# ai-forever/Kandinsky-2

Measured on NVIDIA H100. Metric: unet_denoising_steps_per_sec, higher is better.
Workload: dtype f16

## Files before the change

### kandinsky-2_b200/csrc/k2_api.cu

```cuda
#include <stdio.h>
#include <stdlib.h>
#include <string.h>

#include <algorithm>
#include <atomic>
#include <mutex>

#include "../../include/k2b200.h"
#include "k2_internal.h"

namespace k2 {

static thread_local std::string g_err;
static std::atomic<long long> g_launches{0};
static int g_force_bn = 0;
static int g_force_split = 0;
static int g_pdl = 0;


void set_error(const std::string& msg) { g_err = msg; }
int fail(const std::string& msg) {
  g_err = msg;
  return -1;
}
// ... 74 lines not shown
      const int th = static_cast<int>((H + tiles_h - 1) / tiles_h);
      const long long tiles = tiles_h * tiles_w * ((NB + tn - 1) / tn);
      for (int k = (tn == 1 ? 0 : 1); k < 2; ++k) {
        bool better = best_tiles[k] < 0 || tiles < best_tiles[k];
        if (!better && tiles == best_tiles[k]) {
          if (tn != bn[k]) {
            better = tn < bn[k];
          } else {
            const int d_new = tw > th ? tw - th : th - tw;
            const int d_old = bw[k] > bh[k] ? bw[k] - bh[k] : bh[k] - bw[k];
            better = (d_new < d_old) || (d_new == d_old && tw > bw[k]);
          }
        }
        if (better) {
          best_tiles[k] = tiles;
          bn[k] = tn;
          bw[k] = tw;
          bh[k] = th;
        }
      }
    }
  }
  const int k = (!single_image_only && best_tiles[1] * 100 <= best_tiles[0] * 85) ? 1 : 0;
  TN = bn[k];
  TW = bw[k];
  TH = bh[k];
}


struct ConvPlan {
  int TN, TH, TW, tiles_w, tiles_h, tiles_n, m_tiles;
  int m_tiles_phase;
  int BN, splits;
  int fuse_stats, row_groups;
};

static void plan_conv(int NB, int H, int W, bool any9, int kchunks, int Cout, int out_mode, bool has_workspace,
                      long long workspace_bytes, bool want_gn, ConvPlan& pl, const int* cfg = nullptr, bool up2 = false,
                      bool w_batched = false) {
  const int g_force_bn = (cfg && cfg[0]) ? cfg[0] : k2::g_force_bn;
  const int g_force_split = (cfg && cfg[2]) ? cfg[2] : k2::g_force_split;
  choose_tile(NB, H, W, pl.TN, pl.TH, pl.TW, w_batched);
  pl.tiles_w = (W + pl.TW - 1) / pl.TW;
  pl.tiles_h = (H + pl.TH - 1) / pl.TH;
  pl.tiles_n = (NB + pl.TN - 1) / pl.TN;
  pl.m_tiles = pl.tiles_w * pl.tiles_h * pl.tiles_n;
  pl.m_tiles_phase = pl.m_tiles;

  int BN = g_force_bn;
  int splits = 1;
  const long long M_total = static_cast<long long>(NB) * H * W;
  const bool can_split = !up2 && !w_batched && has_workspace && out_mode == 0 && Cout % 8 == 0;
  auto split_ok = [&](int sp) {
    if (sp == 1) return true;
    const int kps = (kchunks + sp - 1) / sp;
    return can_split && kps >= 8 && (sp - 1) * kps < kchunks &&
           static_cast<long long>(sp) * M_total * Cout * 4 <= workspace_bytes;
  };
  auto model = [&](int bn, int sp) {
    const long long nt = (Cout + bn - 1) / bn;
    const long long units = static_cast<long long>(pl.m_tiles) * nt * sp * (up2 ? 4 : 1);
    const long long slots = num_sms();
    const long long waves = (units + slots - 1) / slots;
    const long long kps = (kchunks + sp - 1) / sp;
    long long cost = waves * (kps * (4LL * bn + 60) + 2000);
    if (sp > 1) cost += 4000 + (static_cast<long long>(sp) + 1) * M_total * Cout * 4 / 1800;
    return cost;
  };
  if (BN == 0) {
    if (Cout <= 16) BN = 16;
    else if (Cout <= 64) BN = 64;
    else if (Cout <= 128) BN = 128;
    else BN = 0;
  }
  {
    const int cand[3] = {256, 192, 128};
    long long best = -1;
    int best_bn = BN ? BN : 256, best_sp = 1;
    for (int ci = 0; ci < 3; ++ci) {
      const int bn = BN ? BN : cand[ci];
      if (BN && ci > 0) break;
      for (int sp = 1; sp <= 8; ++sp) {
        if (g_force_split > 0 && sp != g_force_split) continue;
        if (!split_ok(sp)) continue;
        const long long c = model(bn, sp);
        if (best < 0 || c < best) {
          best = c;
          best_bn = bn;
          best_sp = sp;
        }
      }
    }
    BN = best_bn;
    splits = best_sp;
  }
  pl.BN = BN;
  pl.splits = splits;

  pl.fuse_stats = 0;
  pl.row_groups = 0;
  if (want_gn && out_mode == 0 && Cout % 8 == 0) {
    if (splits == 1 && BN >= 64 && Cout % 64 == 0 && (pl.TN == 1 || pl.TH * pl.TW == 16)) {
      pl.fuse_stats = 1;
      pl.row_groups = ((pl.TN == 1) ? pl.m_tiles : NB * pl.tiles_h * pl.tiles_w) * (up2 ? 4 : 1);
    } else if (splits > 1 && (static_cast<long long>(H) * W) % 16 == 0) {
      pl.fuse_stats = 2;
      pl.row_groups = static_cast<int>(M_total / 16);
    }
  }
}

static void plan_to_info(const ConvPlan& pl, int* info) {
  if (!info) return;
  info[0] = pl.BN; info[1] = 0;
  info[2] = pl.splits; info[3] = pl.m_tiles; info[4] = pl.TN;
  info[5] = pl.fuse_stats; info[6] = pl.row_groups;
}

}

using namespace k2;

extern "C" {

const char* k2_last_error(void) { return g_err.c_str(); }
int k2_version(void) { return 100; }
long long k2_launch_count(void) { return g_launches.load(); }
void k2_reset_launch_count(void) { g_launches.store(0); }
int k2_set_tuning(int key, int value) {
  if (key == 0) {
// ... 16 lines not shown
    return 0;
  }
  if (key == 11) {
    g_gn_bps = value;
    return 0;
  }
  if (key == 9) {
    return 0;
  }

  return fail("k2_set_tuning: unknown key");
}

int k2_conv_gemm(const K2ConvSrc* srcs, int nsrc, int NB, int H, int W, const void* w_packed, int w_rows,
                 int Ktot, int ldw, int Cout, const float* bias, const void* residual, int ldr, void* out, int ldo,
                 int out_mode, void* workspace, long long workspace_bytes, float* gn_partial, int* info,
                 k2_stream_t stream) {
  return k2_conv_gemm_cfg(srcs, nsrc, NB, H, W, w_packed, w_rows, Ktot, ldw, Cout, bias, residual, ldr, out, ldo, out_mode,
                          workspace, workspace_bytes, gn_partial, info, nullptr, 0, stream);
}

int k2_conv_gemm_cfg(const K2ConvSrc* srcs, int nsrc, int NB, int H, int W, const void* w_packed, int w_rows,
                     int Ktot, int ldw, int Cout, const float* bias, const void* residual, int ldr, void* out, int ldo,
                     int out_mode, void* workspace, long long workspace_bytes, float* gn_partial, int* info,
                     const int* cfg, long long w_batch_stride, k2_stream_t stream) {
  K2_REQUIRE(w_batch_stride >= 0 && w_batch_stride % 8 == 0, "conv_gemm_cfg: w_batch_stride must be a multiple of 8 elements");
  K2_REQUIRE(out_mode == 0 || out_mode == 1, "conv_gemm: out_mode must be 0 (fp16 rows) or 1 (fp32 NCHW)");
  K2_REQUIRE(out_mode == 0 || residual == nullptr, "conv_gemm: out_mode 1 (fp32 NCHW) takes no residual");
  const bool w_batched = w_batch_stride > 0;
  if (cfg) {
    K2_REQUIRE(cfg[0] == 0 || cfg[0] == 16 || cfg[0] == 64 || cfg[0] == 128 || cfg[0] == 192 || cfg[0] == 256,
               "conv_gemm_cfg: N tile must be 0, 16, 64, 128, 192 or 256");
    K2_REQUIRE(cfg[1] >= 0 && cfg[1] <= 2 && cfg[2] >= 0 && cfg[2] <= 8 && cfg[3] >= 0 && cfg[3] <= 2,
               "conv_gemm_cfg: pair mode in 0..2, splits in 0..8, epilogue sets in 0..2");
    K2_REQUIRE(cfg[1] != 2, "conv_gemm_cfg: no CTA-pair conv kernel on sm_90");
  }
  K2_REQUIRE(nsrc >= 1 && nsrc <= 3, "conv_gemm: 1..3 sources");
  K2_REQUIRE((reinterpret_cast<uintptr_t>(gn_partial) & 7) == 0, "conv_gemm: gn_partial must be 8-byte aligned");
  K2_REQUIRE(NB > 0 && H > 0 && W > 0 && Cout > 0, "conv_gemm: bad geometry");
  K2_REQUIRE(w_rows >= Cout, "conv_gemm: w_rows < Cout");
  K2_REQUIRE(Ktot % 64 == 0, "conv_gemm: Ktot must be a multiple of 64");
  if (ldw == 0) ldw = Ktot;
  K2_REQUIRE(ldw >= Ktot && ldw % 8 == 0 && (reinterpret_cast<uintptr_t>(w_packed) & 15) == 0,
             "conv_gemm: weight row stride / alignment");
  ConvGemmParams p;
  memset(&p, 0, sizeof p);
  p.NB = NB;
  p.H = H;
  p.W = W;
  bool any9 = false;
  int kchunks = 0;
  const bool up2 = srcs[0].taps == 4;
  if (up2) {
    K2_REQUIRE(nsrc == 1 && out_mode == 0 && residual == nullptr && H % 2 == 0 && W % 2 == 0,
               "conv_gemm: a taps == 4 source (3x3 conv over its nearest-2x upsampling) must be the only source, with fp16 "
               "output, no residual and even output H, W");
    H /= 2;
    W /= 2;
    p.H = H;
    p.W = W;
  }
  for (int s = 0; s < nsrc; ++s) {
    const K2ConvSrc& src = srcs[s];
    K2_REQUIRE(src.taps == 9 || src.taps == 1 || (s == 0 && src.taps == 4), "conv_gemm: taps must be 9 or 1 (or 4: up2)");
    K2_REQUIRE(src.C > 0 && src.C % 8 == 0 && src.ld % 8 == 0 && src.ld >= src.C, "conv_gemm: bad source C/ld");
    K2_REQUIRE((reinterpret_cast<uintptr_t>(src.ptr) & 15) == 0, "conv_gemm: source not 16B aligned");
    any9 = any9 || src.taps == 9;
// ... 27 lines not shown
                        static_cast<uint64_t>(NB)};
    uint64_t str[3] = {static_cast<uint64_t>(src.ld) * 2, static_cast<uint64_t>(src.ld) * 2 * W,
                       static_cast<uint64_t>(src.ld) * 2 * W * H};
    uint32_t box[4] = {64, static_cast<uint32_t>(p.TW), static_cast<uint32_t>(p.TH), static_cast<uint32_t>(p.TN)};
    if (encode_tmap_f16(&p.tmA[s], src.ptr, 4, dims, str, box)) return -1;
  }
  const int BN = pl.BN, splits = pl.splits, fuse_stats = pl.fuse_stats;
  p.splits = splits;
  p.k_per_split = (kchunks + splits - 1) / splits;
  p.M_total = static_cast<long long>(NB) * H * W * (up2 ? 4 : 1);
  p.ws = reinterpret_cast<float*>(workspace);
  p.n_tiles = (Cout + BN - 1) / BN;
  p.Cout = Cout;
  {
    uint64_t dims[3] = {static_cast<uint64_t>(Ktot), static_cast<uint64_t>(w_rows), static_cast<uint64_t>(w_batched ? NB : 1)};
    uint64_t str[2] = {static_cast<uint64_t>(ldw) * 2,
                       (w_batched ? static_cast<uint64_t>(w_batch_stride) : static_cast<uint64_t>(ldw) * w_rows) * 2};
    uint32_t box[3] = {64, static_cast<uint32_t>(BN), 1};
    if (encode_tmap_f16(&p.tmB, w_packed, 3, dims, str, box)) return -1;
  }
  p.bias = bias;
  p.residual = reinterpret_cast<const __half*>(residual);
  p.ldr = ldr;
  p.out = out;
  p.ldo = ldo;
  p.out_mode = (splits > 1) ? 2 : out_mode;
  p.gn_part = (fuse_stats == 1) ? reinterpret_cast<float2*>(gn_partial) : nullptr;
  p.gn_mode = (fuse_stats == 1) ? (p.TN == 1 ? 1 : 2) : 0;
  if (out_mode == 0) {
    K2_REQUIRE(ldo % 8 == 0 && (reinterpret_cast<uintptr_t>(out) & 15) == 0, "conv_gemm: out alignment");
    if (residual)
      K2_REQUIRE(ldr % 8 == 0 && (reinterpret_cast<uintptr_t>(residual) & 15) == 0, "conv_gemm: residual alignment");
  }
  int rc = launch_conv_gemm(p, BN, static_cast<cudaStream_t>(stream));
  if (rc == 0) g_launches.fetch_add(1, std::memory_order_relaxed);
  if (rc == 0 && splits > 1) {
    rc = launch_splitk_finalize(p.ws, splits, p.M_total, Cout, bias, p.residual, ldr, reinterpret_cast<__half*>(out), ldo,
                                fuse_stats == 2 ? reinterpret_cast<float2*>(gn_partial) : nullptr,
                                static_cast<cudaStream_t>(stream));
    if (rc == 0) g_launches.fetch_add(1, std::memory_order_relaxed);
  }
  return rc;
}

int k2_conv_plan(int NB, int H, int W, int taps, int Ktot, int Cout, int out_mode, long long workspace_bytes,
                 int want_gn_partial, int* info) {
  K2_REQUIRE(NB > 0 && H > 0 && W > 0 && Cout > 0 && info, "conv_plan: bad arguments");
  K2_REQUIRE(Ktot > 0 && Ktot % 64 == 0, "conv_plan: Ktot must be a positive multiple of 64");
  ConvPlan pl;
  plan_conv(NB, H, W, taps == 9, Ktot / 64, Cout, out_mode, workspace_bytes > 0, workspace_bytes, want_gn_partial != 0, pl);
  plan_to_info(pl, info);
  return 0;
}

}
```

### kandinsky-2_b200/csrc/k2_conv_gemm.cu

```cuda
#include <stdio.h>

#include "k2_common.cuh"
#include "k2_internal.h"

namespace k2 {

namespace {

constexpr int BM = 128;
constexpr int BK = 64;
constexpr int A_STAGE_BYTES = BM * BK * 2;
constexpr int EPI_WARP_BYTES = 16 * 128;
constexpr int SMEM_LIMIT = 227 * 1024;

template <int BN>
struct Cfg {
  static constexpr int B_STAGE_BYTES = BN * BK * 2;
  static constexpr int STAGE_BYTES = A_STAGE_BYTES + B_STAGE_BYTES;
  static constexpr int EPI_BYTES = 8 * (EPI_WARP_BYTES + BN * 4);
  static constexpr int BAR_BYTES = 256;
  static constexpr int FIXED = EPI_BYTES + BAR_BYTES + 1024;
  static constexpr int STAGES = (SMEM_LIMIT - FIXED) / STAGE_BYTES > 6 ? 6 : (SMEM_LIMIT - FIXED) / STAGE_BYTES;
  static constexpr int SMEM_BYTES = STAGES * STAGE_BYTES + FIXED;
  static_assert(STAGES >= 2, "conv_gemm: shared memory does not hold two pipeline stages");
};

__device__ __forceinline__ void decode_m_tile(const ConvGemmParams& p, int m_idx, int& n0, int& y0,
                                              int& x0, int& phase) {
  phase = 0;
  if (p.up2) {
    phase = m_idx / p.m_tiles_phase;
    m_idx -= phase * p.m_tiles_phase;
  }
  int tw_i = m_idx % p.tiles_w;
  int t = m_idx / p.tiles_w;
  int th_i = t % p.tiles_h;
  int tn_i = t / p.tiles_h;
  x0 = tw_i * p.TW;
  y0 = th_i * p.TH;
  n0 = tn_i * p.TN;
}

__device__ __forceinline__ void ldsm_x4(uint32_t (&r)[4], uint32_t saddr) {
  asm volatile("ldmatrix.sync.aligned.m8n8.x4.shared.b16 {%0, %1, %2, %3}, [%4];"
               : "=r"(r[0]), "=r"(r[1]), "=r"(r[2]), "=r"(r[3])
               : "r"(saddr)
               : "memory");
}

template <int BN>
__device__ __forceinline__ void epilogue_warp(const ConvGemmParams& p, const float (&acc)[BN / 2], float* epi, uint32_t stg,
                                              const float* bsm, int k, int lane, int n0, int y0, int x0, int cbase, int split,
                                              int m_idx, int phase) {
  const int thw = p.TH * p.TW;
  auto out_row_of = [&](int row, int& n, int& y, int& x) -> long long {
    const int tn = row / thw;
    const int rem = row - tn * thw;
    const int th = rem / p.TW;
    const int tw = rem - th * p.TW;
    n = n0 + tn;
    y = y0 + th;
    x = x0 + tw;
    if (tn >= p.TN || n >= p.NB || y >= p.H || x >= p.W) return -1;
    return p.up2 ? (static_cast<long long>(n) * (2 * p.H) + (2 * y + (phase >> 1))) * (2 * p.W) + (2 * x + (phase & 1))
                 : (static_cast<long long>(n) * p.H + y) * p.W + x;
  };
  const int t4 = lane & 3, ra = lane >> 2;
  if constexpr (BN % 64 == 0) {
    if ((p.out_mode == 0 && p.Cout % 64 == 0) || (p.out_mode == 2 && p.Cout % 32 == 0)) {
      int n_, y_, x_;
      const int my_pix = static_cast<int>(out_row_of(16 * k + (lane & 15), n_, y_, x_));
      const int sub = lane >> 3, piece = lane & 7;
      int pix[4];
#pragma unroll
      for (int i = 0; i < 4; ++i) pix[i] = __shfl_sync(0xffffffffu, my_pix, 4 * i + sub);
      const bool va = __shfl_sync(0xffffffffu, my_pix, ra) >= 0, vb = __shfl_sync(0xffffffffu, my_pix, ra + 8) >= 0;
      auto row_addr = [&](int i) {
        const int rr = 4 * i + sub;
        return stg + rr * 128 + ((piece ^ (rr & 7)) << 4);
      };
      const int lrow = (lane & 7) + 8 * ((lane >> 3) & 1);
      auto frag_addr = [&](int q) { return stg + lrow * 128 + (((q + (lane >> 4)) ^ (lane & 7)) << 4); };
      if (p.out_mode == 2) {
        float* wsb = p.ws + static_cast<long long>(split) * p.M_total * p.Cout;
#pragma unroll
        for (int j = 0; j < BN / 32; ++j) {
          const int col0 = cbase + j * 32;
          if (col0 >= p.Cout) break;
#pragma unroll
          for (int q = 0; q < 4; ++q) {
#pragma unroll
            for (int h = 0; h < 2; ++h) {
              const int rr = ra + 8 * h;
              const int i = 16 * j + 4 * q + 2 * h;
              sts_v2(stg + rr * 128 + (((2 * q + (t4 >> 1)) ^ (rr & 7)) << 4) + ((t4 & 1) << 3), __float_as_uint(acc[i]),
                     __float_as_uint(acc[i + 1]));
            }
          }
          __syncwarp();
#pragma unroll
          for (int i = 0; i < 4; ++i) {
            const uint4 v4 = lds_v4(row_addr(i));
            if (pix[i] >= 0)
              *reinterpret_cast<uint4*>(wsb + static_cast<long long>(pix[i]) * p.Cout + col0 + piece * 4) = v4;
          }
          __syncwarp();
        }
        return;
      }
      constexpr int NP = BN / 64;
      const int m_in = p.up2 ? m_idx - phase * p.m_tiles_phase : m_idx;
      auto part_index = [&](long long base) { return p.up2 ? base * 4 + phase : base; };
      __half* outb = reinterpret_cast<__half*>(p.out);
      float4 st[NP];
      uint4 rpre[4];
      auto load_res = [&](int j) {
        const int c0 = cbase + j * 64;
#pragma unroll
        for (int i = 0; i < 4; ++i) {
          rpre[i] = make_uint4(0u, 0u, 0u, 0u);
          if (pix[i] >= 0 && c0 < p.Cout)
            rpre[i] = *reinterpret_cast<const uint4*>(p.residual + static_cast<long long>(pix[i]) * p.ldr + c0 + piece * 8);
        }
      };
      if (p.residual) load_res(0);
#pragma unroll
      for (int j = 0; j < NP; ++j) {
        const int col0 = cbase + j * 64;
        st[j] = make_float4(0.f, 0.f, 0.f, 0.f);
        if (col0 >= p.Cout) continue;
        uint32_t res[16];
        if (p.residual) {
#pragma unroll
          for (int i = 0; i < 4; ++i) sts_v4(row_addr(i), rpre[i].x, rpre[i].y, rpre[i].z, rpre[i].w);
          __syncwarp();
#pragma unroll
          for (int qq = 0; qq < 4; ++qq) {
            uint32_t r4[4];
            ldsm_x4(r4, frag_addr(2 * qq));
#pragma unroll
            for (int m = 0; m < 4; ++m) res[4 * qq + m] = r4[m];
          }
          if (j + 1 < NP) load_res(j + 1);
          __syncwarp();
        }
        uint32_t o[16];
#pragma unroll
// ... 16 lines not shown
          }
        }
#pragma unroll
        for (int qq = 0; qq < 4; ++qq) stmatrix_x4(frag_addr(2 * qq), o[4 * qq], o[4 * qq + 1], o[4 * qq + 2], o[4 * qq + 3]);
        __syncwarp();
#pragma unroll
        for (int i = 0; i < 4; ++i) {
          const uint4 v4 = lds_v4(row_addr(i));
          if (pix[i] >= 0) *reinterpret_cast<uint4*>(outb + static_cast<long long>(pix[i]) * p.ldo + col0 + piece * 8) = v4;
        }
        if (p.gn_part) {
          float4 hs = make_float4(0.f, 0.f, 0.f, 0.f);
#pragma unroll
          for (int rr = 0; rr < 16; ++rr) {
            const uint32_t v = lds_u32(stg + rr * 128 + (((lane >> 2) ^ (rr & 7)) << 4) + ((lane & 3) << 2));
            const float2 t = __half22float2(*reinterpret_cast<const __half2*>(&v));
            hs.x += t.x;
            hs.y = fmaf(t.x, t.x, hs.y);
            hs.z += t.y;
            hs.w = fmaf(t.y, t.y, hs.w);
          }
          if (p.gn_mode == 2) {
            const int per = p.tiles_h * p.tiles_w;
            const int sp = m_in % per;
            const int img = n0 + k;
            if (k < p.TN && img < p.NB)
              *reinterpret_cast<float4*>(p.gn_part + part_index(static_cast<long long>(img) * per + sp) * p.Cout + col0 + 2 * lane) = hs;
          } else {
            st[j] = hs;
          }
        }
        __syncwarp();
      }
      if (p.gn_part && p.gn_mode == 1) {
        float4* sums = reinterpret_cast<float4*>(epi);
#pragma unroll
        for (int j = 0; j < NP; ++j) sums[k * 128 + j * 32 + lane] = st[j];
        named_bar_sync(1, 256);
        if (k < NP && cbase + k * 64 < p.Cout) {
          float4 tot = make_float4(0.f, 0.f, 0.f, 0.f);
#pragma unroll
          for (int e = 0; e < 4; ++e) {
            const float4 a = sums[(2 * e) * 128 + k * 32 + lane], b = sums[(2 * e + 1) * 128 + k * 32 + lane];
            tot.x += a.x + b.x;
            tot.y += a.y + b.y;
            tot.z += a.z + b.z;
            tot.w += a.w + b.w;
          }
          *reinterpret_cast<float4*>(p.gn_part + part_index(m_in) * p.Cout + cbase + k * 64 + 2 * lane) = tot;
        }
        named_bar_sync(1, 256);
      }
      return;
    }
  }
  int n[2], y[2], x[2];
  long long orow[2];
#pragma unroll
  for (int h = 0; h < 2; ++h) orow[h] = out_row_of(16 * k + ra + 8 * h, n[h], y[h], x[h]);
#pragma unroll
  for (int q = 0; q < BN / 8; ++q) {
#pragma unroll
    for (int h = 0; h < 2; ++h) {
#pragma unroll
      for (int e = 0; e < 2; ++e) {
        const int col = cbase + 8 * q + 2 * t4 + e;
        if (orow[h] < 0 || col >= p.Cout) continue;
        float f = acc[4 * q + 2 * h + e];
        if (p.out_mode == 2) {
          p.ws[(static_cast<long long>(split) * p.M_total + orow[h]) * p.Cout + col] = f;
          continue;
        }
        if (p.bias) f += __ldg(p.bias + col);
        if (p.out_mode == 0) {
          if (p.residual) f += __half2float(p.residual[orow[h] * p.ldr + col]);
          reinterpret_cast<__half*>(p.out)[orow[h] * p.ldo + col] = __float2half_rn(f);
        } else {
          reinterpret_cast<float*>(p.out)[((static_cast<long long>(n[h]) * p.Cout + col) * p.H + y[h]) * p.W + x[h]] = f;
        }
      }
    }
  }
}


template <int BN>
__global__ void __launch_bounds__(384, 1) conv_gemm_kernel(const __grid_constant__ ConvGemmParams p) {
  using C = Cfg<BN>;
  constexpr int NA = BN / 2;
  extern __shared__ uint8_t smem_raw[];
  uint8_t* smem = reinterpret_cast<uint8_t*>((reinterpret_cast<uintptr_t>(smem_raw) + 1023) &
                                             ~static_cast<uintptr_t>(1023));
  float* epi = reinterpret_cast<float*>(smem + C::STAGES * C::STAGE_BYTES);
  uint64_t* full_bar = reinterpret_cast<uint64_t*>(smem + C::STAGES * C::STAGE_BYTES + C::EPI_BYTES);
  uint64_t* empty_bar = full_bar + C::STAGES;

  const int warp_idx = threadIdx.x >> 5;
  const int lane = threadIdx.x & 31;
  const int wg = warp_idx >> 2;

  if (threadIdx.x == 0) {
    tma_prefetch_desc(&p.tmB);
    for (int s = 0; s < 3; ++s)
      if (p.seg_taps[s]) tma_prefetch_desc(&p.tmA[s]);
    for (int i = 0; i < C::STAGES; ++i) {
      mbar_init(&full_bar[i], 1);
      mbar_init(&empty_bar[i], 8);
    }
    fence_barrier_init();
  }
  __syncthreads();
  pdl_wait();
  pdl_launch();

  const int total_tiles = p.m_tiles * p.n_tiles * p.splits;

  if (wg == 0) {
    setmaxnreg_dec<40>();
    if (warp_idx == 0 && elect_one()) {
      int stage = 0;
      uint32_t ring_phase = 0;
      const uint32_t tx_bytes = p.a_box_bytes + C::B_STAGE_BYTES;
      for (int tile = blockIdx.x; tile < total_tiles; tile += gridDim.x) {
        const int n_idx = tile % p.n_tiles;
        const int m_idx = (tile / p.n_tiles) % p.m_tiles;
        const int split = tile / (p.m_tiles * p.n_tiles);
        int n0, y0, x0, phase;
        decode_m_tile(p, m_idx, n0, y0, x0, phase);
        const int kb = phase * p.num_k_chunks;
        const int k0 = split * p.k_per_split;
        const int k1 = min(p.num_k_chunks, k0 + p.k_per_split);
        int s = 0, rem = k0;
        while (rem >= p.seg_taps[s] * p.seg_kchunks[s]) {
          rem -= p.seg_taps[s] * p.seg_kchunks[s];
          ++s;
        }
        int tap = rem / p.seg_kchunks[s];
        int c = rem - tap * p.seg_kchunks[s];
        for (int kc = k0; kc < k1; ++kc) {
          const int taps = p.seg_taps[s];
          const int dy = (taps == 9) ? (tap / 3 - 1) : (taps == 4 ? (tap >> 1) + (phase >> 1) - 1 : 0);
          const int dx = (taps == 9) ? (tap % 3 - 1) : (taps == 4 ? (tap & 1) + (phase & 1) - 1 : 0);
          mbar_wait_lean(&empty_bar[stage], ring_phase ^ 1);
          uint8_t* sA = smem + stage * C::STAGE_BYTES;
          uint8_t* sB = sA + A_STAGE_BYTES;
          mbar_arrive_expect_tx(&full_bar[stage], tx_bytes);
          tma_load_4d(sA, &p.tmA[s], &full_bar[stage], c * BK, x0 + dx, y0 + dy, n0);
          tma_load_3d(sB, &p.tmB, &full_bar[stage], (kb + kc) * BK, n_idx * BN, p.w_batched ? n0 : 0);
          if (++stage == C::STAGES) {
            stage = 0;
            ring_phase ^= 1;
          }
          if (++c == p.seg_kchunks[s]) {
            c = 0;
            if (++tap == taps) {
              tap = 0;
              ++s;
            }
          }
        }
      }
    }
  } else {
    setmaxnreg_inc<232>();
    const int g = wg - 1;
    const int k = warp_idx - 4;
    const uint32_t stg = smem_u32(epi) + k * EPI_WARP_BYTES;
    float* bsm = epi + 8 * EPI_WARP_BYTES / 4 + k * BN;
    int bias_cols = -1;
    int stage = 0;
    uint32_t phase = 0;
    for (int tile = blockIdx.x; tile < total_tiles; tile += gridDim.x) {
      const int n_idx = tile % p.n_tiles;
      const int m_idx = (tile / p.n_tiles) % p.m_tiles;
      const int split = tile / (p.m_tiles * p.n_tiles);
      const int nk = min(p.num_k_chunks, (split + 1) * p.k_per_split) - split * p.k_per_split;
      float acc[NA];
#pragma unroll
      for (int i = 0; i < NA; ++i) acc[i] = 0.f;
      int prev_stage = -1;
      for (int kc = 0; kc < nk; ++kc) {
        mbar_wait_lean(&full_bar[stage], phase);
        const uint32_t a_addr = smem_u32(smem + stage * C::STAGE_BYTES) + g * (64 * 128);
        const uint32_t b_addr = smem_u32(smem + stage * C::STAGE_BYTES + A_STAGE_BYTES);
        wgmma_fence();
#pragma unroll
        for (int ks = 0; ks < BK / 16; ++ks) {
          const uint64_t adesc = make_wgmma_desc(a_addr) + static_cast<uint64_t>(ks * 2);
          const uint64_t bdesc = make_wgmma_desc(b_addr) + static_cast<uint64_t>(ks * 2);
          if constexpr (BN == 256) {
            wgmma_m64n256k16(acc, adesc, bdesc, 1u);
          } else if constexpr (BN == 192) {
            wgmma_m64n192k16(acc, adesc, bdesc, 1u);
          } else if constexpr (BN == 128) {
            wgmma_m64n128k16(acc, adesc, bdesc, 1u);
          } else if constexpr (BN == 64) {
            wgmma_m64n64k16(acc, adesc, bdesc, 1u);
          } else {
            static_assert(BN == 16, "conv_gemm: N tile without a wgmma shape");
            wgmma_m64n16k16(acc, adesc, bdesc, 1u);
          }
        }
        wgmma_commit();
        wgmma_wait<1>();
        if (prev_stage >= 0 && lane == 0) mbar_arrive(&empty_bar[prev_stage]);
        prev_stage = stage;
        if (++stage == C::STAGES) {
          stage = 0;
          phase ^= 1;
        }
      }
      wgmma_wait<0>();
#pragma unroll
      for (int i = 0; i < NA; ++i) reg_fence(acc[i]);
      if (prev_stage >= 0 && lane == 0) mbar_arrive(&empty_bar[prev_stage]);

      int n0, y0, x0, mphase;
      decode_m_tile(p, m_idx, n0, y0, x0, mphase);
      const int cbase = n_idx * BN;
      if (p.bias && cbase != bias_cols) {
        __syncwarp();
#pragma unroll
        for (int c = lane; c < BN; c += 32) bsm[c] = (cbase + c < p.Cout) ? __ldg(p.bias + cbase + c) : 0.f;
        __syncwarp();
        bias_cols = cbase;
      }
      epilogue_warp<BN>(p, acc, epi, stg, bsm, k, lane, n0, y0, x0, cbase, split, m_idx, mphase);
    }
  }
}

__global__ void __launch_bounds__(256) splitk_finalize_kernel(const float* __restrict__ ws, int splits, long long M,
                                                              int Cout, const float* __restrict__ bias,
                                                              const __half* __restrict__ residual, int ldr,
                                                              __half* __restrict__ out, int ldo, float2* __restrict__ gn_part) {
  __shared__ float red[8][32][17];
  const int vx = threadIdx.x & 31, ry = threadIdx.x >> 5;
  const int c0 = (blockIdx.y * 32 + vx) * 8;
  const long long rg = blockIdx.x;
  pdl_wait();
  pdl_launch();
  float st[16];
#pragma unroll
  for (int e = 0; e < 16; ++e) st[e] = 0.f;
  if (c0 < Cout) {
    float bv[8];
#pragma unroll
    for (int e = 0; e < 8; ++e) bv[e] = bias ? __ldg(bias + c0 + e) : 0.f;
#pragma unroll
    for (int rr = 0; rr < 2; ++rr) {
      const long long m = rg * 16 + ry + rr * 8;
      if (m >= M) continue;
      float f[8];
#pragma unroll
      for (int e = 0; e < 8; ++e) f[e] = bv[e];
      for (int s = 0; s < splits; ++s) {
        const float4* w = reinterpret_cast<const float4*>(ws + (static_cast<long long>(s) * M + m) * Cout + c0);
        const float4 a = __ldcs(w), b = __ldcs(w + 1);
        f[0] += a.x; f[1] += a.y; f[2] += a.z; f[3] += a.w; f[4] += b.x; f[5] += b.y; f[6] += b.z; f[7] += b.w;
      }
// ... 9 lines not shown
      }
      uint4 ov;
      __half2* oh = reinterpret_cast<__half2*>(&ov);
#pragma unroll
      for (int e = 0; e < 4; ++e) {
        oh[e] = __floats2half2_rn(f[2 * e], f[2 * e + 1]);
        const float2 t = __half22float2(oh[e]);
        st[2 * e] += t.x;
        st[2 * e + 1] += t.y;
        st[8 + 2 * e] = fmaf(t.x, t.x, st[8 + 2 * e]);
        st[8 + 2 * e + 1] = fmaf(t.y, t.y, st[8 + 2 * e + 1]);
      }
      *reinterpret_cast<uint4*>(out + m * ldo + c0) = ov;
    }
  }
  if (gn_part == nullptr) return;
#pragma unroll
  for (int e = 0; e < 16; ++e) red[ry][vx][e] = st[e];
  __syncthreads();
  const int vx2 = threadIdx.x >> 3, e2 = threadIdx.x & 7;
  const int c = (blockIdx.y * 32 + vx2) * 8 + e2;
  if (c < Cout) {
    float s1 = 0.f, s2 = 0.f;
#pragma unroll
    for (int q = 0; q < 8; ++q) {
      s1 += red[q][vx2][e2];
      s2 += red[q][vx2][8 + e2];
    }
    gn_part[rg * Cout + c] = make_float2(s1, s2);
  }
}


template <int BN>
int launch_bn(const ConvGemmParams& p, cudaStream_t stream) {
  using C = Cfg<BN>;
  static bool attr_set = false;
  if (!attr_set) {
    K2_CHECK_CUDA(cudaFuncSetAttribute(conv_gemm_kernel<BN>, cudaFuncAttributeMaxDynamicSharedMemorySize, C::SMEM_BYTES));
    attr_set = true;
  }
  int total = p.m_tiles * p.n_tiles * p.splits;
  int grid = total < num_sms() ? total : num_sms();
  K2_CHECK_CUDA(launch_k(conv_gemm_kernel<BN>, dim3(grid), dim3(384), C::SMEM_BYTES, stream, p));
  return 0;
}

}

int launch_splitk_finalize(const float* ws, int splits, long long M, int Cout, const float* bias, const __half* residual,
                           int ldr, __half* out, int ldo, float2* gn_part, cudaStream_t stream) {
  dim3 grid(static_cast<unsigned int>((M + 15) / 16), (Cout / 8 + 31) / 32);
  K2_CHECK_CUDA(launch_k(splitk_finalize_kernel, grid, dim3(256), 0, stream, ws, splits, M, Cout, bias, residual, ldr, out, ldo,
                         gn_part));
  return 0;
}

int launch_conv_gemm(const ConvGemmParams& p, int BN, cudaStream_t stream) {
  switch (BN) {
    case 16: return launch_bn<16>(p, stream);
    case 64: return launch_bn<64>(p, stream);
    case 128: return launch_bn<128>(p, stream);
    case 192: return launch_bn<192>(p, stream);
    case 256: return launch_bn<256>(p, stream);
    default: return fail("conv_gemm: unsupported BN");
  }
}

}
```

### kandinsky-2_b200/csrc/k2_internal.h

```cpp
#pragma once
#include <cuda.h>
#include <cuda_fp16.h>
#include <cuda_runtime.h>
#include <stdint.h>

#include <string>

namespace k2 {

void set_error(const std::string& msg);
int fail(const std::string& msg);
#define K2_CHECK_CUDA(expr)                                                                 \
  do {                                                                                      \
    cudaError_t _e = (expr);                                                                \
    if (_e != cudaSuccess)                                                                  \
      return ::k2::fail(std::string(#expr) + ": " + cudaGetErrorString(_e));                \
  } while (0)
#define K2_REQUIRE(cond, msg)                                  \
  do {                                                         \
    if (!(cond)) return ::k2::fail(std::string("k2b200: ") + (msg)); \
  } while (0)

inline bool aligned16(const void* p) { return (reinterpret_cast<uintptr_t>(p) & 15) == 0; }

// ... 18 lines not shown
void count_launch(int n = 1);

int encode_tmap_f16(CUtensorMap* out, const void* base, int rank, const uint64_t* dims,
                    const uint64_t* strides_bytes , const uint32_t* box);

struct ConvGemmParams {
  CUtensorMap tmA[3];
  CUtensorMap tmB;
  int w_batched;
  int seg_taps[3];
  int seg_kchunks[3];
  int num_k_chunks;
  int NB, H, W;
  int TN, TH, TW;
  int tiles_n, tiles_h, tiles_w;
  int m_tiles, n_tiles;
  int Cout;
  const float* bias;
  const __half* residual;
  int ldr;
  void* out;
  int ldo;
  int out_mode;
  uint32_t a_box_bytes;
  int splits;
  int k_per_split;
  float* ws;
  long long M_total;
  float2* gn_part;
  int gn_mode;
  int up2;
  int m_tiles_phase;
};
int launch_conv_gemm(const ConvGemmParams& p, int BN, cudaStream_t stream);
int launch_splitk_finalize(const float* ws, int splits, long long M, int Cout, const float* bias, const __half* residual,
                           int ldr, __half* out, int ldo, float2* gn_part, cudaStream_t stream);

struct FlashParams {
  const __half* qkv;
  long long ldq;
  int hs, q_off, k_off, v_off;
  const __half* enc;
  long long lde;
  int ehs, ek_off, ev_off;
  int B, heads, T, Tc;
  __half* out;
  int ldo, ohs;
  float scale_log2e;
};
int gn_apply_blocks_per_sm();
int launch_attention(const FlashParams& p, int head_dim, cudaStream_t stream);

}
```

### kandinsky-2_b200/kandinsky2/launch_plan.py

```python
import gc
import os

import torch

from . import ops

FOLD_MAX_RG = int(os.environ.get("K2_GN_FOLD_MAX_RG", "18"))
TUNE = os.environ.get("K2_AUTOTUNE", "1") != "0"
FORK = os.environ.get("K2_FORK", "1") != "0"
TUNE_SMALL_M = int(os.environ.get("K2_TUNE_SMALL_M", "8192"))
_tune_cache = {}


def tune(key, run, m_rows=0):
    if not TUNE:
        return None
    key = (torch.cuda.current_device(), TUNE_SMALL_M) + key
    if key in _tune_cache:
        return _tune_cache[key]
    info = [0] * 7
    run(None, info)
    bn0, splits = info[0], info[2]
    cout = key[3]
    best = None
    if cout > 64:
        bns = [bn0] if splits > 1 else [bn for bn in (128, 192, 256) if bn - 64 < cout or bn == bn0]
        cands = [(bn0, 0, splits, 1)] + [(bn, 0, splits, 1) for bn in bns if bn != bn0]
        if 0 < m_rows <= TUNE_SMALL_M and splits == 1:
            for bn in (128, 192, 256):
                if bn - 64 >= cout:
                    continue
                for sp in (2, 3, 4):
                    probe = [0] * 7
                    try:
                        run((bn, 1, sp, 1), probe)
                    except Exception:
                        continue
                    if probe[0] == bn and probe[2] == sp:
                        cands.append((bn, 1, sp, 1))

        def timed(cfg, reps=6):
            run(cfg)
            evs = [torch.cuda.Event(enable_timing=True) for _ in range(reps + 1)]
            evs[0].record()
            for i in range(reps):
                run(cfg)
                evs[i + 1].record()
            torch.cuda.synchronize()
            return min(evs[i].elapsed_time(evs[i + 1]) for i in range(reps))

        t0 = tb = timed(cands[0])
        for cfg in cands[1:]:
            t = timed(cfg)
            if t < tb and t < 0.97 * t0:
                t = max(t, timed(cfg))
                if t < tb and t < 0.97 * t0:
                    best, tb = cfg, t
    _tune_cache[key] = best
    return best


class LaunchPlan:
    def __init__(self, dev, nb):
        self.dev = dev
        self.NB = nb
        self._parts = {}
        self._scratch = {}
        self.steps = []
        self.graph = None
        self._side_stream = None
        self._side_open = False
        self._serial = False

# ... 158 lines not shown
```

### profiles/conv_layers.py

```python
import argparse
import json
import os
import subprocess
import sys

ROOT = os.path.dirname(os.path.dirname(os.path.abspath(__file__)))
for p in (ROOT, os.path.join(ROOT, "kandinsky-2_b200")):
    if p not in sys.path:
        sys.path.insert(0, p)

import torch

B, H, W = 4, 96, 96


def _card():
    q = subprocess.run(["nvidia-smi", "--query-gpu=name,power.limit,clocks.max.sm", "--format=csv,noheader", "-i", "0"],
                       capture_output=True, text=True)
    return q.stdout.strip() or torch.cuda.get_device_name(0)


def _pad64(c):
    return (c + 63) // 64 * 64

# ... 79 lines not shown
    tune = launch_plan.tune

    def counting_tune(key, run, m_rows=0):
        counts[key] = counts.get(key, 0) + 1
        return tune(key, run, m_rows=m_rows)
    launch_plan.tune = counting_tune
    model = bench.build_unet(dev)
    image_emb = torch.randn(2 * B, 1280, generator=torch.Generator().manual_seed(1234)).to(dev)
    step = FusedStep(model, B, H, W, dict(image_emb=image_emb), guidance_scale=4.0, cond_first=False, clip_range=2.0,
                     threshold_mode=0)
    launch_plan.tune = tune
    diffusion = create_ddpm_v22(50)
    coef, ts = diffusion._tables(dev)
    order = torch.arange(diffusion.num_timesteps - 1, -1, -1, device=dev)
    step.set_schedule(ts[order], coef[order], torch.randn(len(order), B, 4, H, W, device=dev))
    x = step.latent()
    x.copy_(torch.randn(B, 4, H, W, device=dev))
    step.advance(x)
    torch.cuda.synchronize()
    res["plan_conv_launches"] = sum(1 for _, kind, _ in step.plan.steps if kind == "conv_gemm")
    res["counted_conv_launches"] = sum(counts.values())

    g = torch.Generator(device=dev).manual_seed(7)
    layers = []
    for key, n in counts.items():
        run, shp = _layer(key, dev, g)
        if run is None:
            continue
        info = [0] * 7
        picked = launch_plan._tune_cache.get((dev.index, launch_plan.TUNE_SMALL_M) + key)
        run(picked, info)
        picked_cfg = [info[0], 0, info[2], (picked[3] if picked and picked[3] else 1)]
        cout = shp["N"]
        cfgs = []
        if cout > 64:
            cfgs = [(bn, 0, 1, 1) for bn in (128, 192, 256) if bn - 64 < cout or bn == info[0]]
        if tuple(picked_cfg) not in cfgs:
            cfgs.append(tuple(picked_cfg))
        rows = []
        for cfg in cfgs:
            info = [0] * 7
            run(cfg, info)
            bn, splits = info[0], info[2]
            ms, reps = _time(run, cfg, args.min_ms)
            flops = 2.0 * shp["M"] * cout * shp["K"]
            mma_n = bn if (args.mma_n == "tile" or bn < 64) else 64
            smem_bpf = (2048 + 32 * mma_n) / (2.0 * 64 * mma_n * 16)
            m_tiles = info[3] * (4 if "up2" in shp["desc"] else 1)
            chunks = m_tiles * ((cout + bn - 1) // bn) * (shp["K"] // 64)
            l2_bytes = chunks * (16384 + bn * 128)
            rows.append(dict(n_tile=bn, epilogue_sets=cfg[3], splits=splits, ms=round(ms, 5), reps=reps,
                             tflops=round(flops / (ms * 1e-3) / 1e12, 1),
                             smem_operand_bytes_per_flop=round(smem_bpf, 5),
                             l2_operand_bytes_per_flop=round(l2_bytes / flops, 5),
                             l2_operand_TBps=round(l2_bytes / (ms * 1e-3) / 1e12, 2)))
        pick = next((r for r in rows if [r["n_tile"], r["splits"], r["epilogue_sets"]] ==
                     [picked_cfg[0], picked_cfg[2], picked_cfg[3]]), rows[0])
        layers.append(dict(shape=shp["desc"], key=repr(key), launches_per_step=n, gemm_gflop=round(2e-9 * shp["M"] * cout * shp["K"], 3),
                           picked=dict(n_tile=picked_cfg[0], splits=picked_cfg[2], epilogue_sets=picked_cfg[3],
                                       tuned=picked is not None),
                           picked_ms=pick["ms"], configs=rows))
    total = sum(l["launches_per_step"] * l["picked_ms"] for l in layers)
    for l in layers:
        l["share_of_conv_time"] = round(l["launches_per_step"] * l["picked_ms"] / total, 4)
    layers.sort(key=lambda l: -l["share_of_conv_time"])
    res["conv_ms_per_step_at_picked"] = round(total, 3)
    res["layers"] = layers

    print(f"# {res['card']}  (mma_n={args.mma_n})  conv time per step at the picked configurations: {total:.2f} ms")
    print(f"{'shape':44s} {'n':>2s} {'share':>6s} {'pick':>9s}  " + "  ".join(f"{c:>9s}" for c in
          ("128", "192", "256")) + "   (TFLOP/s at N tile, splits 1)")
    for l in layers:
        by = {(r["n_tile"], r["epilogue_sets"]): r["tflops"] for r in l["configs"] if r["splits"] == 1}
        pk = l["picked"]
        print(f"{l['shape'][:44]:44s} {l['launches_per_step']:2d} {100 * l['share_of_conv_time']:5.1f}% "
              f"{pk['n_tile']:>3d}/{pk['epilogue_sets']}/{pk['splits']:<3d}  " +
              "  ".join(f"{by.get(c, float('nan')):9.1f}" for c in ((128, 1), (192, 1), (256, 1))))
    if args.out:
        os.makedirs(os.path.dirname(os.path.abspath(args.out)), exist_ok=True)
        with open(args.out, "w") as f:
            f.write(json.dumps(res, indent=1) + "\n")


if __name__ == "__main__":
    main()
```

Before: 31.90.

## Add ping-pong warpgroup schedule to conv GEMM kernel and autotune it

Adds a ping-pong variant of the warp-specialized conv GEMM kernel for N tiles up to 128. Each consumer warpgroup now computes a full 128-row tile on alternating tiles, and named barriers order the two groups so one group's epilogue overlaps the other's MMA mainloop. The GroupNorm partial-sum reduction moves into a shared helper that works for both schedules. The autotuner now times the ping-pong schedule as a candidate, including for small-Cout layers. This costs more registers per warpgroup and extra shared memory, and only helps where the tuner selects it.

```diff
diff --git a/kandinsky-2_b200/csrc/k2_api.cu b/kandinsky-2_b200/csrc/k2_api.cu
--- a/kandinsky-2_b200/csrc/k2_api.cu
+++ b/kandinsky-2_b200/csrc/k2_api.cu
@@ -130,6 +130,7 @@
   int TN, TH, TW, tiles_w, tiles_h, tiles_n, m_tiles;
   int m_tiles_phase;
   int BN, splits;
+  int pingpong;
   int fuse_stats, row_groups;
 };
 
@@ -138,6 +139,7 @@
                       bool w_batched = false) {
   const int g_force_bn = (cfg && cfg[0]) ? cfg[0] : k2::g_force_bn;
   const int g_force_split = (cfg && cfg[2]) ? cfg[2] : k2::g_force_split;
+  const int force_sched = cfg ? cfg[3] : 0;
   choose_tile(NB, H, W, pl.TN, pl.TH, pl.TW, w_batched);
   pl.tiles_w = (W + pl.TW - 1) / pl.TW;
   pl.tiles_h = (H + pl.TH - 1) / pl.TH;
@@ -194,6 +196,7 @@
   }
   pl.BN = BN;
   pl.splits = splits;
+  pl.pingpong = BN <= 128 && force_sched == 2;
 
   pl.fuse_stats = 0;
   pl.row_groups = 0;
@@ -276,7 +279,7 @@
     K2_REQUIRE(cfg[0] == 0 || cfg[0] == 16 || cfg[0] == 64 || cfg[0] == 128 || cfg[0] == 192 || cfg[0] == 256,
                "conv_gemm_cfg: N tile must be 0, 16, 64, 128, 192 or 256");
     K2_REQUIRE(cfg[1] >= 0 && cfg[1] <= 2 && cfg[2] >= 0 && cfg[2] <= 8 && cfg[3] >= 0 && cfg[3] <= 2,
-               "conv_gemm_cfg: pair mode in 0..2, splits in 0..8, epilogue sets in 0..2");
+               "conv_gemm_cfg: pair mode in 0..2, splits in 0..8, schedule in 0..2");
     K2_REQUIRE(cfg[1] != 2, "conv_gemm_cfg: no CTA-pair conv kernel on sm_90");
   }
   K2_REQUIRE(nsrc >= 1 && nsrc <= 3, "conv_gemm: 1..3 sources");
@@ -370,7 +373,7 @@
     if (residual)
       K2_REQUIRE(ldr % 8 == 0 && (reinterpret_cast<uintptr_t>(residual) & 15) == 0, "conv_gemm: residual alignment");
   }
-  int rc = launch_conv_gemm(p, BN, static_cast<cudaStream_t>(stream));
+  int rc = launch_conv_gemm(p, BN, pl.pingpong != 0, static_cast<cudaStream_t>(stream));
   if (rc == 0) g_launches.fetch_add(1, std::memory_order_relaxed);
   if (rc == 0 && splits > 1) {
     rc = launch_splitk_finalize(p.ws, splits, p.M_total, Cout, bias, p.residual, ldr, reinterpret_cast<__half*>(out), ldo,
diff --git a/kandinsky-2_b200/csrc/k2_conv_gemm.cu b/kandinsky-2_b200/csrc/k2_conv_gemm.cu
--- a/kandinsky-2_b200/csrc/k2_conv_gemm.cu
+++ b/kandinsky-2_b200/csrc/k2_conv_gemm.cu
@@ -17,7 +17,7 @@
 struct Cfg {
   static constexpr int B_STAGE_BYTES = BN * BK * 2;
   static constexpr int STAGE_BYTES = A_STAGE_BYTES + B_STAGE_BYTES;
-  static constexpr int EPI_BYTES = 8 * (EPI_WARP_BYTES + BN * 4);
+  static constexpr int EPI_BYTES = 8 * (EPI_WARP_BYTES + BN * 4 + (BN <= 128 ? 1024 : 0));
   static constexpr int BAR_BYTES = 256;
   static constexpr int FIXED = EPI_BYTES + BAR_BYTES + 1024;
   static constexpr int STAGES = (SMEM_LIMIT - FIXED) / STAGE_BYTES > 6 ? 6 : (SMEM_LIMIT - FIXED) / STAGE_BYTES;
@@ -49,9 +49,9 @@
 }
 
 template <int BN>
-__device__ __forceinline__ void epilogue_warp(const ConvGemmParams& p, const float (&acc)[BN / 2], float* epi, uint32_t stg,
+__device__ __forceinline__ void epilogue_warp(const ConvGemmParams& p, const float (&acc)[BN / 2], uint32_t stg,
                                               const float* bsm, int k, int lane, int n0, int y0, int x0, int cbase, int split,
-                                              int m_idx, int phase) {
+                                              int m_idx, int phase, float4 (&st)[BN >= 64 ? BN / 64 : 1]) {
   const int thw = p.TH * p.TW;
   auto out_row_of = [&](int row, int& n, int& y, int& x) -> long long {
     const int tn = row / thw;
@@ -112,7 +112,6 @@
       const int m_in = p.up2 ? m_idx - phase * p.m_tiles_phase : m_idx;
       auto part_index = [&](long long base) { return p.up2 ? base * 4 + phase : base; };
       __half* outb = reinterpret_cast<__half*>(p.out);
-      float4 st[NP];
       uint4 rpre[4];
       auto load_res = [&](int j) {
         const int c0 = cbase + j * 64;
@@ -195,25 +194,6 @@
         }
         __syncwarp();
       }
-      if (p.gn_part && p.gn_mode == 1) {
-        float4* sums = reinterpret_cast<float4*>(epi);
-#pragma unroll
-        for (int j = 0; j < NP; ++j) sums[k * 128 + j * 32 + lane] = st[j];
-        named_bar_sync(1, 256);
-        if (k < NP && cbase + k * 64 < p.Cout) {
-          float4 tot = make_float4(0.f, 0.f, 0.f, 0.f);
-#pragma unroll
-          for (int e = 0; e < 4; ++e) {
-            const float4 a = sums[(2 * e) * 128 + k * 32 + lane], b = sums[(2 * e + 1) * 128 + k * 32 + lane];
-            tot.x += a.x + b.x;
-            tot.y += a.y + b.y;
-            tot.z += a.z + b.z;
-            tot.w += a.w + b.w;
-          }
-          *reinterpret_cast<float4*>(p.gn_part + part_index(m_in) * p.Cout + cbase + k * 64 + 2 * lane) = tot;
-        }
-        named_bar_sync(1, 256);
-      }
       return;
     }
   }
@@ -246,15 +226,47 @@
   }
 }
 
-
-template <int BN>
+template <int BN, bool PP>
+__device__ __forceinline__ void gn_fold(const ConvGemmParams& p, float* epi, const float4* gsum, int g, int k, int lane,
+                                        int cbase, int m_idx, int phase, const float4 (&st)[BN / 64]) {
+  constexpr int NP = BN / 64;
+  float4* stage_sums = reinterpret_cast<float4*>(epi);
+  const int w = PP ? k & 3 : k;
+  auto slot = [&](int r, int j) -> const float4* {
+    if (!PP) return stage_sums + r * 128 + j * 32 + lane;
+    return (r < 4 ? gsum + (4 * g + r) * 64 : stage_sums + (4 * g + r - 4) * 128) + j * 32 + lane;
+  };
+#pragma unroll
+  for (int j = 0; j < NP; ++j) stage_sums[k * 128 + j * 32 + lane] = st[j];
+  const int bar = PP ? 1 + g : 1, nthreads = PP ? 128 : 256;
+  named_bar_sync(bar, nthreads);
+  if (w < NP && cbase + w * 64 < p.Cout) {
+    float4 tot = make_float4(0.f, 0.f, 0.f, 0.f);
+#pragma unroll
+    for (int e = 0; e < 4; ++e) {
+      const float4 a = *slot(2 * e, w), b = *slot(2 * e + 1, w);
+      tot.x += a.x + b.x;
+      tot.y += a.y + b.y;
+      tot.z += a.z + b.z;
+      tot.w += a.w + b.w;
+    }
+    const long long row = p.up2 ? static_cast<long long>(m_idx - phase * p.m_tiles_phase) * 4 + phase : m_idx;
+    *reinterpret_cast<float4*>(p.gn_part + row * p.Cout + cbase + w * 64 + 2 * lane) = tot;
+  }
+  named_bar_sync(bar, nthreads);
+}
+
+template <int BN, bool PP>
 __global__ void __launch_bounds__(384, 1) conv_gemm_kernel(const __grid_constant__ ConvGemmParams p) {
+  static_assert(!PP || BN <= 128, "conv_gemm: a 128 x BN fp32 ping-pong tile must fit one warpgroup's registers");
   using C = Cfg<BN>;
   constexpr int NA = BN / 2;
+  constexpr int NST = BN >= 64 ? BN / 64 : 1;
   extern __shared__ uint8_t smem_raw[];
   uint8_t* smem = reinterpret_cast<uint8_t*>((reinterpret_cast<uintptr_t>(smem_raw) + 1023) &
                                              ~static_cast<uintptr_t>(1023));
   float* epi = reinterpret_cast<float*>(smem + C::STAGES * C::STAGE_BYTES);
+  float4* gsum = reinterpret_cast<float4*>(epi + 8 * EPI_WARP_BYTES / 4 + 8 * BN);
   uint64_t* full_bar = reinterpret_cast<uint64_t*>(smem + C::STAGES * C::STAGE_BYTES + C::EPI_BYTES);
   uint64_t* empty_bar = full_bar + C::STAGES;
 
@@ -268,7 +280,7 @@
       if (p.seg_taps[s]) tma_prefetch_desc(&p.tmA[s]);
     for (int i = 0; i < C::STAGES; ++i) {
       mbar_init(&full_bar[i], 1);
-      mbar_init(&empty_bar[i], 8);
+      mbar_init(&empty_bar[i], PP ? 4 : 8);
     }
     fence_barrier_init();
   }
@@ -328,6 +340,7 @@
     setmaxnreg_inc<232>();
     const int g = wg - 1;
     const int k = warp_idx - 4;
+    const int w = k & 3;
     const uint32_t stg = smem_u32(epi) + k * EPI_WARP_BYTES;
     float* bsm = epi + 8 * EPI_WARP_BYTES / 4 + k * BN;
     int bias_cols = -1;
@@ -338,13 +351,25 @@
       const int m_idx = (tile / p.n_tiles) % p.m_tiles;
       const int split = tile / (p.m_tiles * p.n_tiles);
       const int nk = min(p.num_k_chunks, (split + 1) * p.k_per_split) - split * p.k_per_split;
-      float acc[NA];
+      if constexpr (PP) {
+        const int it = tile / gridDim.x;
+        if ((it & 1) != g) {
+          const int pos = stage + max(nk, 0);
+          stage = pos % C::STAGES;
+          phase ^= (pos / C::STAGES) & 1;
+          continue;
+        }
+        if (it > 0) named_bar_sync(g ? 3 : 4, 256);
+      }
+      float acc[NA], acc1[PP ? NA : 1];
 #pragma unroll
       for (int i = 0; i < NA; ++i) acc[i] = 0.f;
-      int prev_stage = -1;
+#pragma unroll
+      for (int i = 0; i < (PP ? NA : 1); ++i) acc1[i] = 0.f;
+      int prev_stage = -1, prev2_stage = -1, prev3_stage = -1;
       for (int kc = 0; kc < nk; ++kc) {
         mbar_wait_lean(&full_bar[stage], phase);
-        const uint32_t a_addr = smem_u32(smem + stage * C::STAGE_BYTES) + g * (64 * 128);
+        const uint32_t a_addr = smem_u32(smem + stage * C::STAGE_BYTES) + (PP ? 0 : g * (64 * 128));
         const uint32_t b_addr = smem_u32(smem + stage * C::STAGE_BYTES + A_STAGE_BYTES);
         wgmma_fence();
 #pragma unroll
@@ -357,38 +382,68 @@
             wgmma_m64n192k16(acc, adesc, bdesc, 1u);
           } else if constexpr (BN == 128) {
             wgmma_m64n128k16(acc, adesc, bdesc, 1u);
+            if constexpr (PP) wgmma_m64n128k16(acc1, make_wgmma_desc(a_addr + 64 * 128) + static_cast<uint64_t>(ks * 2), bdesc, 1u);
           } else if constexpr (BN == 64) {
             wgmma_m64n64k16(acc, adesc, bdesc, 1u);
+            if constexpr (PP) wgmma_m64n64k16(acc1, make_wgmma_desc(a_addr + 64 * 128) + static_cast<uint64_t>(ks * 2), bdesc, 1u);
           } else {
             static_assert(BN == 16, "conv_gemm: N tile without a wgmma shape");
             wgmma_m64n16k16(acc, adesc, bdesc, 1u);
+            if constexpr (PP) wgmma_m64n16k16(acc1, make_wgmma_desc(a_addr + 64 * 128) + static_cast<uint64_t>(ks * 2), bdesc, 1u);
           }
         }
         wgmma_commit();
-        wgmma_wait<1>();
-        if (prev_stage >= 0 && lane == 0) mbar_arrive(&empty_bar[prev_stage]);
+        if constexpr (PP) {
+          wgmma_wait<3>();
+          if (prev3_stage >= 0 && lane == 0) mbar_arrive(&empty_bar[prev3_stage]);
+          prev3_stage = prev2_stage;
+          prev2_stage = prev_stage;
+        } else {
+          wgmma_wait<1>();
+          if (prev_stage >= 0 && lane == 0) mbar_arrive(&empty_bar[prev_stage]);
+        }
         prev_stage = stage;
         if (++stage == C::STAGES) {
           stage = 0;
           phase ^= 1;
         }
       }
+      if (PP && tile + gridDim.x < total_tiles) named_bar_arrive(g ? 4 : 3, 256);
       wgmma_wait<0>();
 #pragma unroll
       for (int i = 0; i < NA; ++i) reg_fence(acc[i]);
-      if (prev_stage >= 0 && lane == 0) mbar_arrive(&empty_bar[prev_stage]);
+#pragma unroll
+      for (int i = 0; i < (PP ? NA : 1); ++i) reg_fence(acc1[i]);
+      if (lane == 0) {
+        if (prev3_stage >= 0) mbar_arrive(&empty_bar[prev3_stage]);
+        if (prev2_stage >= 0) mbar_arrive(&empty_bar[prev2_stage]);
+        if (prev_stage >= 0) mbar_arrive(&empty_bar[prev_stage]);
+      }
 
       int n0, y0, x0, mphase;
       decode_m_tile(p, m_idx, n0, y0, x0, mphase);
       const int cbase = n_idx * BN;
-      if (p.bias && cbase != bias_cols) {
+      if (p.bias && (PP || cbase != bias_cols)) {
         __syncwarp();
 #pragma unroll
         for (int c = lane; c < BN; c += 32) bsm[c] = (cbase + c < p.Cout) ? __ldg(p.bias + cbase + c) : 0.f;
         __syncwarp();
         bias_cols = cbase;
       }
-      epilogue_warp<BN>(p, acc, epi, stg, bsm, k, lane, n0, y0, x0, cbase, split, m_idx, mphase);
+      float4 st[NST];
+      epilogue_warp<BN>(p, acc, stg, bsm, PP ? w : k, lane, n0, y0, x0, cbase, split, m_idx, mphase, st);
+      if constexpr (PP) {
+        if constexpr (BN % 64 == 0) {
+          if (p.gn_part && p.gn_mode == 1) {
+#pragma unroll
+            for (int j = 0; j < NST; ++j) gsum[k * 64 + j * 32 + lane] = st[j];
+          }
+        }
+        epilogue_warp<BN>(p, acc1, stg, bsm, w + 4, lane, n0, y0, x0, cbase, split, m_idx, mphase, st);
+      }
+      if constexpr (BN % 64 == 0) {
+        if (p.gn_part && p.gn_mode == 1) gn_fold<BN, PP>(p, epi, gsum, g, k, lane, cbase, m_idx, mphase, st);
+      }
     }
   }
 }
@@ -464,17 +519,17 @@
 }
 
 
-template <int BN>
+template <int BN, bool PP>
 int launch_bn(const ConvGemmParams& p, cudaStream_t stream) {
   using C = Cfg<BN>;
   static bool attr_set = false;
   if (!attr_set) {
-    K2_CHECK_CUDA(cudaFuncSetAttribute(conv_gemm_kernel<BN>, cudaFuncAttributeMaxDynamicSharedMemorySize, C::SMEM_BYTES));
+    K2_CHECK_CUDA(cudaFuncSetAttribute(conv_gemm_kernel<BN, PP>, cudaFuncAttributeMaxDynamicSharedMemorySize, C::SMEM_BYTES));
     attr_set = true;
   }
   int total = p.m_tiles * p.n_tiles * p.splits;
   int grid = total < num_sms() ? total : num_sms();
-  K2_CHECK_CUDA(launch_k(conv_gemm_kernel<BN>, dim3(grid), dim3(384), C::SMEM_BYTES, stream, p));
+  K2_CHECK_CUDA(launch_k(conv_gemm_kernel<BN, PP>, dim3(grid), dim3(384), C::SMEM_BYTES, stream, p));
   return 0;
 }
 
@@ -488,13 +543,21 @@
   return 0;
 }
 
-int launch_conv_gemm(const ConvGemmParams& p, int BN, cudaStream_t stream) {
+int launch_conv_gemm(const ConvGemmParams& p, int BN, bool pingpong, cudaStream_t stream) {
+  if (pingpong) {
+    switch (BN) {
+      case 16: return launch_bn<16, true>(p, stream);
+      case 64: return launch_bn<64, true>(p, stream);
+      case 128: return launch_bn<128, true>(p, stream);
+      default: return fail("conv_gemm: no ping-pong schedule above N tile 128");
+    }
+  }
   switch (BN) {
-    case 16: return launch_bn<16>(p, stream);
-    case 64: return launch_bn<64>(p, stream);
-    case 128: return launch_bn<128>(p, stream);
-    case 192: return launch_bn<192>(p, stream);
-    case 256: return launch_bn<256>(p, stream);
+    case 16: return launch_bn<16, false>(p, stream);
+    case 64: return launch_bn<64, false>(p, stream);
+    case 128: return launch_bn<128, false>(p, stream);
+    case 192: return launch_bn<192, false>(p, stream);
+    case 256: return launch_bn<256, false>(p, stream);
     default: return fail("conv_gemm: unsupported BN");
   }
 }
diff --git a/kandinsky-2_b200/csrc/k2_internal.h b/kandinsky-2_b200/csrc/k2_internal.h
--- a/kandinsky-2_b200/csrc/k2_internal.h
+++ b/kandinsky-2_b200/csrc/k2_internal.h
@@ -74,7 +74,7 @@
   int up2;
   int m_tiles_phase;
 };
-int launch_conv_gemm(const ConvGemmParams& p, int BN, cudaStream_t stream);
+int launch_conv_gemm(const ConvGemmParams& p, int BN, bool pingpong, cudaStream_t stream);
 int launch_splitk_finalize(const float* ws, int splits, long long M, int Cout, const float* bias, const __half* residual,
                            int ldr, __half* out, int ldo, float2* gn_part, cudaStream_t stream);
 
diff --git a/kandinsky-2_b200/kandinsky2/launch_plan.py b/kandinsky-2_b200/kandinsky2/launch_plan.py
--- a/kandinsky-2_b200/kandinsky2/launch_plan.py
+++ b/kandinsky-2_b200/kandinsky2/launch_plan.py
@@ -23,22 +23,22 @@
     bn0, splits = info[0], info[2]
     cout = key[3]
     best = None
-    if cout > 64:
-        bns = [bn0] if splits > 1 else [bn for bn in (128, 192, 256) if bn - 64 < cout or bn == bn0]
-        cands = [(bn0, 0, splits, 1)] + [(bn, 0, splits, 1) for bn in bns if bn != bn0]
-        if 0 < m_rows <= TUNE_SMALL_M and splits == 1:
-            for bn in (128, 192, 256):
-                if bn - 64 >= cout:
+    scheds = lambda bn: (1, 2) if bn <= 128 else (1,)
+    bns = [bn0] if splits > 1 or cout <= 64 else [bn for bn in (128, 192, 256) if bn - 64 < cout or bn == bn0]
+    cands = [(bn, 0, splits, s) for bn in [bn0] + [bn for bn in bns if bn != bn0] for s in scheds(bn)]
+    if cout > 64 and 0 < m_rows <= TUNE_SMALL_M and splits == 1:
+        for bn in (128, 192, 256):
+            if bn - 64 >= cout:
+                continue
+            for sp in (2, 3, 4):
+                probe = [0] * 7
+                try:
+                    run((bn, 1, sp, 1), probe)
+                except Exception:
                     continue
-                for sp in (2, 3, 4):
-                    probe = [0] * 7
-                    try:
-                        run((bn, 1, sp, 1), probe)
-                    except Exception:
-                        continue
-                    if probe[0] == bn and probe[2] == sp:
-                        cands.append((bn, 1, sp, 1))
-
+                if probe[0] == bn and probe[2] == sp:
+                    cands += [(bn, 1, sp, s) for s in scheds(bn)]
+    if len(cands) > 1:
         def timed(cfg, reps=6):
             run(cfg)
             evs = [torch.cuda.Event(enable_timing=True) for _ in range(reps + 1)]
diff --git a/profiles/conv_layers.py b/profiles/conv_layers.py
--- a/profiles/conv_layers.py
+++ b/profiles/conv_layers.py
@@ -135,9 +135,8 @@
         run(picked, info)
         picked_cfg = [info[0], 0, info[2], (picked[3] if picked and picked[3] else 1)]
         cout = shp["N"]
-        cfgs = []
-        if cout > 64:
-            cfgs = [(bn, 0, 1, 1) for bn in (128, 192, 256) if bn - 64 < cout or bn == info[0]]
+        bns = [bn for bn in (128, 192, 256) if bn - 64 < cout or bn == info[0]] if cout > 64 else [info[0]]
+        cfgs = [(bn, 0, 1, s) for bn in bns for s in ((1, 2) if bn <= 128 else (1,))]
         if tuple(picked_cfg) not in cfgs:
             cfgs.append(tuple(picked_cfg))
         rows = []
@@ -152,15 +151,15 @@
             m_tiles = info[3] * (4 if "up2" in shp["desc"] else 1)
             chunks = m_tiles * ((cout + bn - 1) // bn) * (shp["K"] // 64)
             l2_bytes = chunks * (16384 + bn * 128)
-            rows.append(dict(n_tile=bn, epilogue_sets=cfg[3], splits=splits, ms=round(ms, 5), reps=reps,
+            rows.append(dict(n_tile=bn, schedule=cfg[3], splits=splits, ms=round(ms, 5), reps=reps,
                              tflops=round(flops / (ms * 1e-3) / 1e12, 1),
                              smem_operand_bytes_per_flop=round(smem_bpf, 5),
                              l2_operand_bytes_per_flop=round(l2_bytes / flops, 5),
                              l2_operand_TBps=round(l2_bytes / (ms * 1e-3) / 1e12, 2)))
-        pick = next((r for r in rows if [r["n_tile"], r["splits"], r["epilogue_sets"]] ==
+        pick = next((r for r in rows if [r["n_tile"], r["splits"], r["schedule"]] ==
                      [picked_cfg[0], picked_cfg[2], picked_cfg[3]]), rows[0])
         layers.append(dict(shape=shp["desc"], key=repr(key), launches_per_step=n, gemm_gflop=round(2e-9 * shp["M"] * cout * shp["K"], 3),
-                           picked=dict(n_tile=picked_cfg[0], splits=picked_cfg[2], epilogue_sets=picked_cfg[3],
+                           picked=dict(n_tile=picked_cfg[0], splits=picked_cfg[2], schedule=picked_cfg[3],
                                        tuned=picked is not None),
                            picked_ms=pick["ms"], configs=rows))
     total = sum(l["launches_per_step"] * l["picked_ms"] for l in layers)
@@ -172,13 +171,13 @@
 
     print(f"# {res['card']}  (mma_n={args.mma_n})  conv time per step at the picked configurations: {total:.2f} ms")
     print(f"{'shape':44s} {'n':>2s} {'share':>6s} {'pick':>9s}  " + "  ".join(f"{c:>9s}" for c in
-          ("128", "192", "256")) + "   (TFLOP/s at N tile, splits 1)")
+          ("128/coop", "128/pp", "192", "256")) + "   (TFLOP/s at N tile / schedule, splits 1)")
     for l in layers:
-        by = {(r["n_tile"], r["epilogue_sets"]): r["tflops"] for r in l["configs"] if r["splits"] == 1}
+        by = {(r["n_tile"], r["schedule"]): r["tflops"] for r in l["configs"] if r["splits"] == 1}
         pk = l["picked"]
         print(f"{l['shape'][:44]:44s} {l['launches_per_step']:2d} {100 * l['share_of_conv_time']:5.1f}% "
-              f"{pk['n_tile']:>3d}/{pk['epilogue_sets']}/{pk['splits']:<3d}  " +
-              "  ".join(f"{by.get(c, float('nan')):9.1f}" for c in ((128, 1), (192, 1), (256, 1))))
+              f"{pk['n_tile']:>3d}/{pk['schedule']}/{pk['splits']:<3d}  " +
+              "  ".join(f"{by.get(c, float('nan')):9.1f}" for c in ((128, 1), (128, 2), (192, 1), (256, 1))))
     if args.out:
         os.makedirs(os.path.dirname(os.path.abspath(args.out)), exist_ok=True)
         with open(args.out, "w") as f:
```

Result: no change. 31.84, median of 6 (-0.2%).
